# TUM-DAML/gemnet_pytorch

Hardware: AMD Instinct MI355X
Metric: molecules/sec (forward+force) GemNet-T on COLL-shaped batches (higher is better)
Workload: dtype f32

## Files before the change

gemnet_pytorch_amd/csrc/atom_stack.hip:

```cpp
#include <type_traits>

#include "common.h"

#include "chain_split.h"

#pragma clang fp contract(off)

#ifndef AS_EXP
#define AS_EXP 0
#endif

#ifndef AS_AHEAD
#define AS_AHEAD 2
#endif

namespace {
using namespace gn_split;

__device__ __forceinline__ float as_fma(float a, float b, float c) { return __builtin_fmaf(a, b, c); }

__device__ __forceinline__ void as_ssilu_pair(float x, float& y, float& d) {
  const float s = gn_sigmoid(x), xs = x * s;
  const float t = s + xs;
  d = as_fma(-s, xs, t) * GN_INV_06;
// ... 33 lines not shown

  uint4 w[NG][4][2];
  auto wload = [&](auto jc) {
    constexpr int j = decltype(jc)::value;
    if constexpr (j < NG) {
      const uint4* __restrict__ const base = P.W[j] + (size_t)wave * (4 * 2 * 64) + lane;
#pragma unroll
      for (int c = 0; c < 4; ++c)
#pragma unroll
        for (int p = 0; p < 2; ++p) w[j][c][p] = AS_EXP == 1 ? make_uint4(0x3c003c00u + lane, 0u, 0u, 0u) : base[(c * 2 + p) * 64];
    }
  };
  const int lr = tid >> 5, lc = (tid & 31) << 2;
  float4 xv = make_float4(0.f, 0.f, 0.f, 0.f);
  if (row0 + lr < M) xv = *reinterpret_cast<const float4*>(P.x + (size_t)(row0 + lr) * SW + lc);
  wload(std::integral_constant<int, 0>{});
  if constexpr (AS_AHEAD > 1) wload(std::integral_constant<int, 1>{});
  if constexpr (AS_AHEAD > 2) wload(std::integral_constant<int, 2>{});
  if constexpr (AS_AHEAD > 3) wload(std::integral_constant<int, 3>{});
  if constexpr (AS_AHEAD > 4) wload(std::integral_constant<int, 4>{});
  if constexpr (AS_AHEAD > 5) wload(std::integral_constant<int, 5>{});
  if constexpr (AS_AHEAD > 6) wload(std::integral_constant<int, 6>{});

  auto plane_ptr = [&](int slot, int p) -> unsigned char* { return smem + slot * SLOT + p * PLANE; };
  auto sw_off = [&](int row, int col) -> int { return row * ROWB + ((((col >> 3) ^ row) & 15) << 4) + ((col & 4) << 1); };
  auto slot_write = [&](int slot, int row, int col, const float4 v) {
    const int off = sw_off(row, col);
    uint2 H, Lo;
    split4h(v, H, Lo);
    *reinterpret_cast<uint2*>(plane_ptr(slot, 0) + off) = H;
    *reinterpret_cast<uint2*>(plane_ptr(slot, 1) + off) = Lo;
  };

  slot_write(0, lr, lc, xv);
  lds_barrier();

  const int n0 = wave * 16 + (lg << 2);
  const bool ok = row0 + l15 < M;
  const uint32_t off = (uint32_t)(row0 + l15) * (uint32_t)SW + (uint32_t)n0;
  const int my = sw_off(l15, n0);

  auto gemm = [&](auto jc) {
    constexpr int j = decltype(jc)::value;
    constexpr bool tail = j >= NM;
    constexpr bool second = !tail && j > 0 && (j & 1) == 0;
    constexpr bool last = j == NM - 1;
    constexpr int a_slot = tail ? 1 : (j & 1);
    constexpr int y_slot = a_slot ^ 1;
    uint4 xf[4][2];
    {
      const unsigned char* xb = smem + a_slot * SLOT + l15 * ROWB;
#pragma unroll
      for (int c = 0; c < 4; ++c) {
        const unsigned char* xp = xb + ((((c << 2) | lg) ^ l15) << 4);
        xf[c][0] = *reinterpret_cast<const uint4*>(xp);
        xf[c][1] = *reinterpret_cast<const uint4*>(xp + PLANE);
      }
    }
    uint2 rH = make_uint2(0u, 0u), rL = make_uint2(0u, 0u);
    if constexpr (second) {
      rH = *reinterpret_cast<const uint2*>(plane_ptr(y_slot, 0) + my);
      rL = *reinterpret_cast<const uint2*>(plane_ptr(y_slot, 1) + my);
    }
    float4 q2 = make_float4(0.f, 0.f, 0.f, 0.f);
    if constexpr (last && RES2) {
      if (ok) q2 = *reinterpret_cast<const float4*>(P.res2 + off);
    }
    v4f acc[3];
#pragma unroll
    for (int k = 0; k < 3; ++k) acc[k] = (v4f){0.f, 0.f, 0.f, 0.f};
#pragma unroll
    for (int c = 0; c < 4; ++c) {
      const f16x8 ah = __builtin_bit_cast(f16x8, w[j][c][0]), al = __builtin_bit_cast(f16x8, w[j][c][1]);
      const f16x8 yh = __builtin_bit_cast(f16x8, xf[c][0]), yl = __builtin_bit_cast(f16x8, xf[c][1]);
      if constexpr (AS_EXP == 3) {
        acc[0][0] += __uint_as_float(w[j][c][0].x ^ xf[c][0].x); acc[1][0] += __uint_as_float(w[j][c][0].y ^ xf[c][1].y);
        acc[2][0] += __uint_as_float(w[j][c][1].z ^ xf[c][0].z);
        continue;
      }
      acc[0] = __builtin_amdgcn_mfma_f32_16x16x32_f16(ah, yh, acc[0], 0, 0, 0);
      acc[1] = __builtin_amdgcn_mfma_f32_16x16x32_f16(ah, yl, acc[1], 0, 0, 0);
      acc[2] = __builtin_amdgcn_mfma_f32_16x16x32_f16(al, yh, acc[2], 0, 0, 0);
    }
    const v4f corr = acc[1] + acc[2];
    float4 v = make_float4(as_fma(corr[0], H_DOWN, acc[0][0]), as_fma(corr[1], H_DOWN, acc[0][1]),
                           as_fma(corr[2], H_DOWN, acc[0][2]), as_fma(corr[3], H_DOWN, acc[0][3]));
    wload(std::integral_constant<int, j + AS_AHEAD>{});
    if constexpr (tail) {
      if (ok) *reinterpret_cast<float4*>(P.t[j - NM] + off) = v;
    } else {
      float4 d;
      if constexpr (AS_EXP == 2) {
        d = v;
      } else {
        as_ssilu_pair(v.x, v.x, d.x); as_ssilu_pair(v.y, v.y, d.y);
        as_ssilu_pair(v.z, v.z, d.z); as_ssilu_pair(v.w, v.w, d.w);
      }
      if (ok) *reinterpret_cast<float4*>(P.z[j] + off) = d;
      if constexpr (second) {
        const float4 q = join4h(rH, rL);
        const float b = P.s;
        v.x = (v.x + q.x) * b; v.y = (v.y + q.y) * b; v.z = (v.z + q.z) * b; v.w = (v.w + q.w) * b;
      }
      if constexpr (last && RES2) {
        if (ok) {
          const float b = P.beta2;
          v.x = (v.x + q2.x) * b; v.y = (v.y + q2.y) * b; v.z = (v.z + q2.z) * b; v.w = (v.w + q2.w) * b;
        }
      }
      if constexpr (last) {
        if (ok) *reinterpret_cast<float4*>(P.y + off) = v;
      }
      if constexpr (!last || T > 0) {
        slot_write(y_slot, l15, n0, ok ? v : make_float4(0.f, 0.f, 0.f, 0.f));
        if constexpr (AS_EXP != 4) lds_barrier();
      }
    }
  };
  gemm(std::integral_constant<int, 0>{});
  if constexpr (NG > 1) gemm(std::integral_constant<int, 1>{});
  if constexpr (NG > 2) gemm(std::integral_constant<int, 2>{});
  if constexpr (NG > 3) gemm(std::integral_constant<int, 3>{});
  if constexpr (NG > 4) gemm(std::integral_constant<int, 4>{});
  if constexpr (NG > 5) gemm(std::integral_constant<int, 5>{});
  if constexpr (NG > 6) gemm(std::integral_constant<int, 6>{});
}

template <int L, int T, bool RES2>
int launch_fwd(const as_fwd_args& a, hipStream_t st) {
  hipLaunchKernelGGL((atom_stack_fwd_kernel<L, T, RES2>), dim3((unsigned)gn_cdiv(a.M, 16)), dim3(NT), 0, st, a);
  GN_LAUNCH_CHECK();
  return 0;
}

template <int L, int T>
int launch_fwd_res(const as_fwd_args& a, hipStream_t st) {
  if constexpr (L > 0) {
    if (a.res2) return launch_fwd<L, T, true>(a, st);
  }
  return launch_fwd<L, T, false>(a, st);
}

template <int L>
int launch_fwd_tails(const as_fwd_args& a, int tails, hipStream_t st) {
  switch (tails) {
    case 0: return launch_fwd_res<L, 0>(a, st);
    case 1: return launch_fwd_res<L, 1>(a, st);
    default: return launch_fwd_res<L, 2>(a, st);
  }
}

bool aligned16(const void* p) { return (reinterpret_cast<uintptr_t>(p) & 15u) == 0; }

}

extern "C" int gn_atom_stack_fwd_f32(const float* x, int M, int layers, int tails, const void* const* W, float* const* z,
                                     float s, const float* res2, float beta2, float* y, float* const* t, void* stream) {
  if (M <= 0) return 0;
  if (M > AS_MAX_ROWS || layers < 0 || layers > 2 || tails < 0 || tails > 2) return (int)hipErrorInvalidValue;
  if (!x || !y || !W || !z || (tails && !t) || (res2 && layers == 0)) return (int)hipErrorInvalidValue;
  if (!aligned16(x) || !aligned16(y) || !aligned16(res2)) return (int)hipErrorInvalidValue;
  as_fwd_args a = {};
  a.x = x; a.M = M; a.s = s; a.res2 = res2; a.beta2 = beta2; a.y = y;
  const int nm = 1 + 2 * layers;
  for (int j = 0; j < nm + tails; ++j) {
    if (!W[j] || !aligned16(W[j])) return (int)hipErrorInvalidValue;
    a.W[j] = static_cast<const uint4*>(W[j]);
  }
  for (int j = 0; j < nm; ++j) {
    if (!z[j] || !aligned16(z[j])) return (int)hipErrorInvalidValue;
    a.z[j] = z[j];
  }
  for (int j = 0; j < tails; ++j) {
    if (!t[j] || !aligned16(t[j])) return (int)hipErrorInvalidValue;
    a.t[j] = t[j];
  }
  hipStream_t st = static_cast<hipStream_t>(stream);
  switch (layers) {
    case 0: return launch_fwd_tails<0>(a, tails, st);
    case 1: return launch_fwd_tails<1>(a, tails, st);
    default: return launch_fwd_tails<2>(a, tails, st);
  }
}
```

gemnet_pytorch_amd/kernels.py:

```python
import contextlib
import ctypes
import functools
import os
import threading

import torch

from . import _lib
from ._lib import (GN_ANG_F16, GN_CHAIN_MAX_OPS, GN_CHAIN_ROW, GN_SPLIT_F16X2_ROW, GemmArgs, addr, check, ptr,
                   require_device, stream)


def _f32c(t):
    if t.dtype != torch.float32:
        raise TypeError(f"HIP path is fp32; got {t.dtype}")
    return t.contiguous()


def _rowmajor(t):
    if t.dtype != torch.float32:
        raise TypeError(f"HIP path is fp32; got {t.dtype}")
    if t.dim() != 2:
        raise ValueError("2-D operand expected")
    if t.shape[0] > 0 and t.shape[1] > 0 and t.stride(1) == 1 and t.stride(0) >= t.shape[1]:
# ... 1288 lines not shown


_CHAIN_PACK = None


def _chain_packer():
    global _CHAIN_PACK
    if _CHAIN_PACK is None:
        import struct
        from ._lib import ChainArgs, ChainOp
        code = {ctypes.c_int: "i", ctypes.c_float: "f", ctypes.c_void_p: "P"}
        names, fmt = [], "@"
        for name, ct in ChainOp._fields_:
            names.append(name)
            fmt += code[ct]
        st = struct.Struct(fmt)
        probe = bytearray(ctypes.sizeof(ChainOp))
        vals = list(range(1, len(names) + 1))
        st.pack_into(probe, 0, *[float(v) if c == ctypes.c_float else v for v, (_, c) in zip(vals, ChainOp._fields_)])
        chk = ChainOp.from_buffer_copy(bytes(probe))
        assert all(getattr(chk, n) == (float(v) if c == ctypes.c_float else v)
                   for v, (n, c) in zip(vals, ChainOp._fields_)) and st.size <= ctypes.sizeof(ChainOp)
        default = [0.0 if c == ctypes.c_float else 0 for _, c in ChainOp._fields_]
        for i, n in enumerate(names):
            globals()["F_" + n] = i
            if n in ("slot", "a_slot", "mul_slot", "res_slot", "res2_slot", "y2_slot"):
                default[i] = -1
        _CHAIN_PACK = (st, default, ChainArgs.ops.offset, ctypes.sizeof(ChainOp), ctypes.sizeof(ChainArgs),
                       struct.Struct("@ii"))
    return _CHAIN_PACK


def _mat(t, cols=None):
    if not (t.is_cuda and t.dtype == torch.float32 and t.dim() == 2 and t.is_contiguous()):
        require_device(t)
        raise AssertionError("chain operands: contiguous fp32 2-D")
    if cols is not None and t.shape[1] != cols:
        raise AssertionError((tuple(t.shape), cols))
    return addr(t)


def _source(v, src, stage, cols):
    v[F_src_stage], v[F_src_mode], v[F_src_alpha] = stage, int(src["mode"]), float(src["alpha"])
    v[F_srcP] = _mat(src["P"], cols)
    v[F_srcQ] = _mat(src["Q"], cols) if src["Q"] is not None else 0


GROUP_TILE_ROWS = int(os.environ.get("GN_CHAIN_GROUP_TILE_ROWS", "0"))


def pack_weight_split_stacked(Ws, trans=False, fmt=None):
    if fmt is None:
        fmt = split_format() or 0
    W0 = Ws[0]
    N, Kd = (W0.shape[1], W0.shape[0]) if trans else (W0.shape[0], W0.shape[1])
    nbytes = -(-N // 16) * -(-Kd // 32) * (2 if fmt else 3) * 64 * 16
    out = torch.empty((len(Ws), nbytes), device=W0.device, dtype=torch.uint8)
    for g, W in enumerate(Ws):
        require_device(W)
        W = _rowmajor(W)
        assert tuple(W.shape) == tuple(W0.shape)
        check(_lib.load().gn_pack_weight_split_fmt(ptr(W), N, Kd, W.stride(0), int(bool(trans)), int(fmt), ptr(out[g]), stream()),
              "gn_pack_weight_split_fmt")
    out._gn_fmt = fmt
    return out


def chain_grouped_supported(mode=None):
    return (mode or current_mode()) in ("h3", "split6") and CHAIN_LAYOUT == "tall"


USE_ATOM_STACK = os.environ.get("GEMNET_ATOM_STACK", "1") == "1"
ATOM_STACK_MAX_ROWS = 4096
ATOM_STACK_WIDTH = 128


def _atom_mat(t, M):
    return (torch.is_tensor(t) and t.dtype == torch.float32 and tuple(t.shape) == (M, ATOM_STACK_WIDTH)
            and t.is_contiguous() and t.data_ptr() % 16 == 0)


def _atom_gemm_plain(o):
    return (o["kind"] == "gemm" and tuple(o["W"].shape) == (ATOM_STACK_WIDTH, ATOM_STACK_WIDTH) and o["alpha"] == 1.0
            and o["gadd1"] is None and o["gadd2"] is None and o["mul"] is None and o["res_rows"] is None
            and o["y2"] < 0 and o["Z2"] is None and o["out2"] is None and o.get("add") is None and o.get("add2") is None)


def atom_stack_match(prog, mode=None):
    M, ops = prog.M, prog.ops
    if not (1 <= M <= ATOM_STACK_MAX_ROWS) or (mode or current_mode()) != "h3" or CHAIN_LAYOUT != "tall":
        return None
    if len(ops) < 2 or len(ops) > 8:
        return None
    o = ops[0]
    if not (o["kind"] == "load" and o["slot"] == 0 and o["rows"] is None and o.get("alpha", 1.0) == 1.0 and o.get("y2", -1) < 0
            and o.get("Z2") is None and o.get("add2") is None and _atom_mat(o["src"], M)):
        return None
    n_main = 0
    while 1 + n_main < len(ops) and ops[1 + n_main]["kind"] == "gemm" and ops[1 + n_main]["slot"] >= 0:
        n_main += 1
    main, tails = ops[1:1 + n_main], ops[1 + n_main:]
    L = (n_main - 1) // 2
    if n_main not in (1, 3, 5) or len(tails) > 2:
        return None
    s, res2, beta2 = 1.0, None, 1.0
    for j, g in enumerate(main):
        last = j + 1 == len(main)
        if not (_atom_gemm_plain(g) and g["act"] and g.get("pre_deriv") and _atom_mat(g["pre_out"], M)
                and g["a_slot"] == (j & 1) and g["slot"] == 1 - (j & 1)):
            return None
        if (g["out"] is not None) != last or (last and not _atom_mat(g["out"], M)):
            return None
        second = j > 0 and j % 2 == 0
        if second:
            if not (isinstance(g["res"], int) and g["res"] == 1 and (j == 2 or g["beta"] == s)):
                return None
            s = g["beta"]
        elif g["res"] is not None:
            return None
        if g["res2"] is not None:
            if not (second and last and _atom_mat(g["res2"], M)):
                return None
            res2, beta2 = g["res2"], g["beta2"]
    for g in tails:
        if not (_atom_gemm_plain(g) and not g["act"] and g["a_slot"] == 1 and g["slot"] < 0 and g["pre_out"] is None
                and g["res"] is None and g["res2"] is None and _atom_mat(g["out"], M)):
            return None
    return dict(x=ops[0]["src"], L=L, gemms=main + tails, z=[g["pre_out"] for g in main], s=s, res2=res2, beta2=beta2,
                y=main[-1]["out"], t=[g["out"] for g in tails])


def _atom_stack_fwd(M, m):
    fmt = SPLIT_FORMAT["h3"]
    require_device(m["x"], m["y"], m["res2"], *m["z"], *m["t"])
    Ws = []
    for g in m["gemms"]:
        Wp = g.get("packed")
        if Wp is None:
            _mat(g["W"])
            Wp = pack_weight_split(g["W"], fmt=fmt)
        elif getattr(Wp, "_gn_fmt", 0) != fmt:
            raise RuntimeError(f"chain: weight planes packed in format {getattr(Wp, '_gn_fmt', 0)} handed to a launch in "
                               f"mode 'h3' (format {fmt})")
        Ws.append(Wp)
    z, t = m["z"], m["t"]
    arr = ctypes.c_void_p
    check(_lib.load().gn_atom_stack_fwd_f32(ptr(m["x"]), int(M), int(m["L"]), len(t), (arr * len(Ws))(*[addr(W) for W in Ws]),
                                            (arr * len(z))(*[addr(a) for a in z]), float(m["s"]), ptr(m["res2"]),
                                            float(m["beta2"]), ptr(m["y"]), (arr * max(1, len(t)))(*[addr(a) for a in t]),
                                            stream()),
          "gn_atom_stack_fwd_f32")


def chain(prog, mode=None, groups=0, group_pitch=0, tile_rows=None):
    from ._lib import GN_OP_GEMM, GN_OP_LOAD, GN_OP_SCALE, GN_OP_STORE
    ops = prog.ops
    if len(ops) > GN_CHAIN_MAX_OPS:
        raise ValueError("chain program too long")
    mode = mode or current_mode()
    if USE_ATOM_STACK and not groups and prog.M <= ATOM_STACK_MAX_ROWS:
        m = atom_stack_match(prog, mode)
        if m is not None:
            return _atom_stack_fwd(prog.M, m)
    nprod = CHAIN_MODES[mode]
    if nprod and not chain_split_supported(prog):
        nprod = 0
    if groups and not (nprod and chain_grouped_supported(mode)):
        raise RuntimeError(f"chain: no grouped launch in mode {mode!r} / layout {CHAIN_LAYOUT!r} for this program")
    fmt = SPLIT_FORMAT.get(mode, 0)
    row = nprod == CHAIN_MODES["h3"] and CHAIN_LAYOUT == "row"
    if row and not chain_row_supported(prog):
        raise RuntimeError("chain: the row-resident layout needs K and every width to be a multiple of 16 "
                           "(GEMNET_CHAIN_LAYOUT=tall runs other shapes)")
    if row:
        fmt = GN_SPLIT_F16X2_ROW
    if nprod == CHAIN_MODES["h3"] and not row and h3_hazards(prog):
        raise RuntimeError("chain: this linear program adds a global tensor into an LDS-resident value "
                           f"(ops {h3_hazards(prog)}): not representable in the row-scaled fp16 form 'h3' — "
                           "launch it in kernels.linear_mode('h3')")
    st, default, ops_off, op_size, args_size, hdr = _chain_packer()
    keep = []
    buf = bytearray(args_size)
    M = prog.M
    hdr.pack_into(buf, 0, M, len(ops))
    has_src = False
    off = ops_off
    for o in ops:
        v = default[:]
        kind = o["kind"]
        if kind == "gemm":
            W = o["W"]
            N, Kd = W.shape
            if nprod:
                Wp = o.get("packed")
                if Wp is None:
                    _mat(W)
                    Wp = pack_weight_split(W, fmt=fmt)
                elif getattr(Wp, "_gn_fmt", 0) != fmt:
                    raise RuntimeError(f"chain: weight planes packed in format {getattr(Wp, '_gn_fmt', 0)} handed to a "
                                       f"launch in mode {mode!r} (format {fmt})")
                keep.append(Wp)
                v[F_W] = addr(Wp)
            else:
                v[F_W] = _mat(W)
            v[F_kind], v[F_N], v[F_K], v[F_a_slot], v[F_slot] = GN_OP_GEMM, N, Kd, o["a_slot"], o["slot"]
            v[F_act], v[F_alpha], v[F_beta], v[F_beta2] = int(o["act"]) | (2 if o.get("pre_deriv") else 0), o["alpha"], o["beta"], o["beta2"]
            if o.get("pre_deriv") and not nprod:
                raise RuntimeError("chain: pre_deriv needs the split-operand kernel (not CHAIN_MODE 'f32')")
            t = o["gadd1"]
            if t is not None:
                v[F_gadd1], v[F_gidx1] = _mat(t, N), addr(o["gidx1"])
            t = o["gadd2"]
            if t is not None:
                v[F_gadd2], v[F_gidx2] = _mat(t, N), addr(o["gidx2"])
            t = o["pre_out"]
            if t is not None:
                v[F_pre_out] = _mat(t, N)
            t = o["out"]
            if t is not None:
                v[F_out] = _mat(t, N)
            t = o["mul"]
            if t is not None:
                if isinstance(t, int):
                    v[F_mul_slot] = t
                else:
                    v[F_mul_g] = _mat(t, N)
            t = o["res"]
            if t is not None:
                if isinstance(t, int):
                    v[F_res_slot] = t
                else:
                    v[F_res_g] = _mat(t, N)
            t = o["res2"]
            if t is not None:
                if isinstance(t, int):
                    v[F_res2_slot] = t
                else:
                    v[F_res2_g] = _mat(t, N)
            t = o["res_rows"]
            if t is not None:
                v[F_res_rows] = addr(t)
            mm = o["mul_mode"]
            v[F_mul_mode], v[F_y2_slot], v[F_y2_src], v[F_mode2], v[F_alpha2] = mm, o["y2"], o["y2_src"], o["mode2"], o["alpha2"]
            t = o["Z2"]
            if t is not None:
                v[F_Z2] = _mat(t, N)
            t = o["out2"]
            if t is not None:
                v[F_out2] = _mat(t, N)
            if mm > 1:
                assert v[F_mul_slot] < 0 and v[F_mul_g], "mul_mode applies to a global mul operand"
            t = o.get("add")
            if t is not None:
                _source(v, t, 1, N)
                has_src = True
            t = o.get("add2")
            if t is not None:
                _source(v, t, 2, N)
                has_src = True
        elif kind == "load":
            src = o["src"]
            sp = _mat(src)
            assert o["rows"] is not None or src.shape[0] == M
            w = src.shape[1]
            v[F_kind], v[F_slot], v[F_width], v[F_ld], v[F_src] = GN_OP_LOAD, o["slot"], w, src.stride(0), sp
            t = o["rows"]
            if t is not None:
                v[F_rows] = addr(t)
            v[F_alpha], v[F_y2_slot], v[F_alpha2], v[F_mode2] = o.get("alpha", 1.0), o.get("y2", -1), o.get("alpha2", 1.0), o.get("mode2", 0)
            t = o.get("Z2")
            if t is not None:
                v[F_Z2] = _mat(t, w)
            t = o.get("add2")
            if t is not None:
                _source(v, t, 2, w)
                has_src = True
        elif kind == "scale":
            Z, out = o["Z"], o["out"]
            w = o["width"] or (Z.shape[1] if Z is not None else out.shape[1])
            v[F_kind], v[F_slot], v[F_a_slot], v[F_width], v[F_ld] = GN_OP_SCALE, o["slot"], o["a_slot"], w, w
            v[F_alpha], v[F_act] = o["alpha"], o.get("mode", 0)
            if Z is not None:
                v[F_src] = _mat(Z, w)
            if out is not None:
                v[F_out] = _mat(out, w)
            t = o.get("add")
            if t is not None:
                _source(v, t, 1, w)
                has_src = True
        else:
            out = o["out"]
            v[F_kind], v[F_slot], v[F_width], v[F_ld], v[F_out] = GN_OP_STORE, o["slot"], out.shape[1], out.stride(0), _mat(out)
        st.pack_into(buf, off, *v)
        off += op_size
    if has_src and not nprod:
        raise RuntimeError("chain programs with second-order source terms run on the split-operand kernel only "
                           "(CHAIN_MODE f32 / an unsupported shape): use the composite training path")
    cbuf = (ctypes.c_char * args_size).from_buffer(buf)
    if row:
        nprod |= GN_CHAIN_ROW
    if groups:
        if _lib.TRACE is not None:
            reads, writes = [], []
            for o in ops:
                for key, t in o.items():
                    if key == "packed" and t is not None:
                        reads.append((t.data_ptr(), t.numel() * t.element_size()))
                    elif torch.is_tensor(t) and key not in ("W", "packed") and t.dim() == 2:
                        span = ((int(groups) - 1) * int(group_pitch) + t.shape[0]) * t.stride(0) * t.element_size()
                        (writes if key in ("pre_out", "out", "out2") else reads).append((t.data_ptr(), span))
            _lib.note(reads=reads, writes=writes)
        check(_lib.load().gn_chain_split_grouped_f32(ctypes.addressof(cbuf), nprod, int(groups), int(group_pitch),
                                                     GROUP_TILE_ROWS if tile_rows is None else int(tile_rows), stream()),
              "gn_chain_split_grouped_f32")
    elif nprod:
        check(_lib.load().gn_chain_split_f32(ctypes.addressof(cbuf), nprod, stream()), "gn_chain_split_f32")
# ... 286 lines not shown
```

include/gemnet_hip.h:

```cpp
#ifndef GEMNET_HIP_H
#define GEMNET_HIP_H

#include <stdint.h>

#ifdef __cplusplus
extern "C" {
#endif

int gn_abi_version(void);
const char* gn_error_string(int code);

typedef struct {
  const float* A; const float* B; float* C;
  int M, N, K;
  int lda, ldb, ldc;
  int trans_a, trans_b;
  const float* a_dact_pre;
  int act;
  float* pre_out;
  const float* mul; int ldmul;
  float alpha;
  const float* res; int ldres;
  float beta;
  const float* gadd1; const int32_t* gidx1;
  const float* gadd2; const int32_t* gidx2;
  int ldg;
  const int32_t* ridx;
  const float* res2; int ldres2;
  float beta2;
  float* splitk_ws; int splitk;
} gn_gemm_args;
int gn_gemm_f32(const gn_gemm_args* args, void* stream);
int gn_gemm_f32_cfg(const gn_gemm_args* args, int cfg, void* stream);

enum { GN_OP_LOAD = 0, GN_OP_SCALE = 1, GN_OP_GEMM = 2, GN_OP_STORE = 3 };
#define GN_CHAIN_MAX_OPS 20
typedef struct {
  int kind;
  int slot;
  int a_slot;
  int width;
  int ld;
  const float* src;
  const int32_t* rows;
  const float* W; int N; int K;
  int act;
  float alpha;
  const float* gadd1; const int32_t* gidx1;
  const float* gadd2; const int32_t* gidx2;
  float* pre_out;
  int mul_slot; const float* mul_g;
  int res_slot; const float* res_g; const int32_t* res_rows; float beta;
  int res2_slot; const float* res2_g; float beta2;
  float* out;
  int mul_mode;
  int y2_slot;
  int y2_src;
  int mode2;
  float alpha2;
  const float* Z2;
  float* out2;
  int src_stage;
  int src_mode;
  float src_alpha;
  const float* srcP;
  const float* srcQ;
} gn_chain_op;
typedef struct {
  int M;
  int n_ops;
  gn_chain_op ops[GN_CHAIN_MAX_OPS];
} gn_chain_args;
int gn_chain_f32(const gn_chain_args* args, void* stream);

#define GN_CHAIN_F16X2 2
#define GN_CHAIN_ROW 0x200
int gn_chain_split_f32(const gn_chain_args* args, int nprod, void* stream);
#define GN_CHAIN_MAX_GROUPS 8
#define GN_CHAIN_GROUP_TILE_ROWS 32
int gn_chain_split_grouped_f32(const gn_chain_args* args, int nprod, int groups, int group_pitch, int tile_rows, void* stream);
int gn_atom_stack_fwd_f32(const float* x, int M, int layers, int tails, const void* const* W, float* const* z, float s,
                          const float* res2, float beta2, float* y, float* const* t, void* stream);
int gn_pack_weight_split(const float* W, int N, int K, int ldw, int trans, void* out, void* stream);
#define GN_SPLIT_BF16X3 0
#define GN_SPLIT_F16X2 1
#define GN_SPLIT_F16X2_ROW 2
int gn_pack_weight_split_fmt(const float* W, int N, int K, int ldw, int trans, int fmt, void* out, void* stream);
int64_t gn_pack_weight_split_bytes(int N, int K);
typedef struct {
  const float* W; void* out;
  int N, K, ldw, trans, unit_begin, fmt;
} gn_pack_job;
int gn_pack_weight_split_grouped(const gn_pack_job* jobs, int n_jobs, int total_units, void* stream);

int gn_gemm_tn_f32(const float* A, const float* B, float* C, int M, int N, int K, int lda, int ldb, int ldc,
                   float alpha, float* ws, int splitk, void* stream);
int gn_gemm_tn_splitk(int M, int N, int K);

typedef struct {
  const float* X; const float* Y;
  int M, N, K, ldx, ldy, splitk, kchunk, wg_begin;
  int64_t ws_off;
  float alpha;
  int pad_;
} gn_tn_problem;
typedef struct {
  float* out;
  int64_t n;
  int slice_begin, slice_end, wg_begin;
  int cols;
  int ld, pad_;
} gn_tn_target;
int gn_gemm_tn_grouped_f32(const gn_tn_problem* probs, int n_prob, int total_wg, const gn_tn_target* targets,
                           int n_target, int total_fold_wg, const int64_t* slice_off, float* ws, void* stream);

int gn_rbf_aggregate_fwd_f32(const float* m, const float* rbf, const float* W, const int32_t* perm, const int32_t* seg_off,
                             float* out, int64_t n_atoms, int C, int R, float scale, void* stream);
int gn_rbf_aggregate_bwd_f32(const float* g_out, const float* m, const float* rbf, const float* W, const int32_t* id_a,
                             float* g_m, float* g_rbf, int64_t E, int C, int R, float scale, int accum, void* stream);

#define GN_AGG_MAX_GROUPS 8
int gn_rbf_aggregate_grouped_fwd_f32(const float* const* m_list, const float* const* W_list, const float* scales, int G,
                                     const float* rbf, const int32_t* perm, const int32_t* seg_off, float* out, int64_t n_atoms,
                                     int C, int R, void* stream);
int gn_rbf_aggregate_grouped_bwd_f32(const float* g_out, const float* const* m_list, const float* const* W_list,
                                     const float* scales, int G, const float* rbf, const int32_t* id_a, float* const* g_m_list,
                                     float* g_rbf, int64_t E, int64_t n_atoms, int C, int R, int accum_m, int accum_rbf,
                                     void* stream);

int gn_energy_head_fwd_f32(const float* x, const float* w, float* E, int G, int64_t n_atoms, int C, void* stream);
int gn_energy_head_bwd_f32(const float* g_E, const float* w, float* g_x, int G, int64_t n_atoms, int C, void* stream);

int gn_quad_angles_fwd_f32(const float* R, const int32_t* qc, const int32_t* qa, const int32_t* qb, const int32_t* qd,
                           float* ang, int64_t Q, void* stream);
int gn_quad_angles_bwd_ld_f32(const float* g_ang, const float* R, const int32_t* qc, const int32_t* qa, const int32_t* qb,
                              const int32_t* qd, float* Gc, int ldc, float* Gb, int ldb, float* Gd, int ldd, int64_t Q,
                              void* stream);
#define GN_ANG_F16 1
int gn_bil_reduce_project_ang_f32(const float* ang, const float* x, const int32_t* expand_idx, const int32_t* seg_off,
                                  const float* B, float* Sm, float* P, int64_t E, int S, int C, int I, int arith,
                                  void* stream);
int gn_bil_expand_ang_f32(const float* ang, const float* dSm, const int32_t* seg_off, float* dxt, int64_t E, int S, int C,
                          int arith, void* stream);
int gn_bil_expand_rows_ang_f32(const float* ang, const float* dSm, const int32_t* a_perm, const int32_t* a_seg,
                               const int32_t* j_off, const int32_t* qmap, const int32_t* g_off, const int32_t* task_atom,
                               const int32_t* task_row0, int64_t n_tasks, float* dx, int S, int C, int arith, void* stream);
int gn_quad_angles_jvp_f32(const float* R, const float* tR, const int32_t* qc, const int32_t* qa, const int32_t* qb,
                           const int32_t* qd, float* tang, int64_t Q, void* stream);
int gn_bil_reduce_project_ang_tan_f32(const float* ang, const float* tang, const float* x, const float* tx,
                                      const int32_t* expand_idx, const int32_t* seg_off, const float* B, const float* tB,
                                      const float* Sm, float* Smd, float* Pd, int64_t E, int S, int C, int I, void* stream);
int gn_bil_expand_ang_tan_f32(const float* ang, const float* tang, const float* D1, const float* D2, const int32_t* seg_off,
                              float* dxt, int64_t E, int S, int C, void* stream);
int gn_bil_expand_rows_ang_tan_f32(const float* ang, const float* tang, const float* D1, const float* D2, const int32_t* a_perm,
                                   const int32_t* a_seg, const int32_t* j_off, const int32_t* qmap, const int32_t* g_off,
                                   const int32_t* task_atom, const int32_t* task_row0, int64_t n_tasks, float* dx, int S, int C,
                                   int tile, void* stream);
int gn_bil_dy_multi_ang_f32(const float* const* dSm_list, const float* const* x_list, int nb, const float* ang,
                            const int32_t* expand_idx, const int32_t* seg_off, float* g_ang, int64_t E, int S, int C,
                            int arith, void* stream);

int gn_bmm_f32(const float* A, const float* B, float* C, int batch, int m, int n, int k,
               int trans_a, int trans_b, void* stream);

int64_t gn_index_gpu_ws_bytes(int A, int64_t sum_n2, int triplets_only);
int gn_index_gpu_stage1(const void* R, int r_is_f64, const int32_t* mol_off, const int32_t* sq_off, int B, int A,
                        int nmax, int64_t sum_n2, double cutoff, double int_cutoff, int triplets_only, void* ws,
                        int32_t* batch_seg, int32_t* id_a, int32_t* id_c, int32_t* id_undir, int32_t* id_swap,
                        int32_t* id4_int_a, int32_t* id4_int_b, int64_t* sizes, void* stream);
int gn_index_gpu_stage2(const int32_t* mol_off, const int32_t* sq_off, int B, int A, int64_t sum_n2,
                        int triplets_only, void* ws, const int32_t* id_a, const int32_t* id_c,
                        const int32_t* id4_int_a, const int32_t* id4_int_b, int64_t E, int64_t Eint,
                        int32_t* id3_reduce_ca, int32_t* id3_expand_ba, int32_t* Kidx3, int32_t* id4_reduce_ca,
                        int32_t* id4_expand_db, int32_t* id4_reduce_cab, int32_t* id4_expand_abd, int32_t* Kidx4,
                        int32_t* id4_reduce_intm_ca, int32_t* id4_expand_intm_db, int32_t* id4_reduce_intm_ab,
                        int32_t* id4_expand_intm_ab, void* stream);

int gn_index_gpu_padded_t(const void* R, int r_is_f64, const int32_t* mol_off, const int32_t* sq_off, int B, int A, int nmax,
                          int64_t sum_n2, double cutoff, void* ws, int e_cap, int t_cap, int a_cap, int n_groups,
                          int deg_bound, int32_t* staging, int32_t* id_c, int32_t* id_a, int32_t* id_swap, int32_t* id_undir,
                          int32_t* id3_reduce_ca, int32_t* id3_expand_ba, int32_t* state, void* stream);
int gn_index_poison_f32(float* x, int64_t n, const int32_t* state, void* stream);
int gn_index_gpu_padded_q(const void* R, int r_is_f64, const int32_t* mol_off, const int32_t* sq_off, int B, int A, int nmax,
                          int64_t sum_n2, double cutoff, double int_cutoff, void* ws, int e_cap, int t_cap, int eint_cap,
                          int i_cap, int q_cap, int a_cap, int n_groups, int deg_bound, int32_t* staging, int32_t* const* arrays,
                          int32_t* state, void* stream);

int gn_gather_rows_f32(const float* x, const int32_t* idx, float* y, int64_t T, int C, void* stream);
int gn_gather_mul_f32(const float* x, const int32_t* idx, const float* m, float* y, int64_t T, int C, float scale,
                      void* stream);
int gn_segsum_rows_f32(const float* y, const int32_t* perm, const int32_t* seg_off, float* x,
                       int64_t N, int C, void* stream);
int gn_segsum_pair_f32(const float* y, const int32_t* perm1, const int32_t* seg_off1, float* x1, int64_t N1,
                       const int32_t* perm2, const int32_t* seg_off2, float* x2, int64_t N2, int C, void* stream);
int gn_segsum_multi_f32(int n_terms, const float* const* y, const int32_t* const* perm, const int32_t* const* seg_off,
                        const float* sign, float* x, int64_t N, int C, void* stream);

int64_t gn_csr_ws_bytes(int64_t n, int64_t n_rows);
int gn_csr_build_i32(const int32_t* keys, int64_t n, int64_t n_rows, int32_t* perm, int32_t* seg_off, void* ws,
                     int64_t ws_bytes, void* stream);
int gn_seg_offsets_i32(const int32_t* sorted_keys, int64_t n, int64_t n_rows, int32_t* seg_off, void* stream);
int gn_expanded_csr_i32(const int32_t* perm_e, const int32_t* seg_e, int64_t n_rows, const int32_t* seg_off_of_edge, int64_t E,
                        int32_t* perm, int32_t* seg_out, int32_t* ws, void* stream);

int gn_bil_reduce_f32(const float* Y, const float* x, const int32_t* expand_idx,
                      const int32_t* seg_off, float* Sm, int64_t E, int S, int C, void* stream);
int gn_bil_reduce_t_f32(const float* Y, const float* dSm, const int32_t* reduce_idx,
                        const int32_t* permT, const int32_t* segT_off, float* dx,
                        int64_t J, int S, int C, void* stream);
int gn_bil_reduce_t_grouped_f32(const float* Y, const float* dSm, const int32_t* grp_rows, const int32_t* grp_off,
                                const int32_t* grp_kseg, const int32_t* permT, const int32_t* rposT, float* dx,
                                int64_t G, int max_rows, int S, int C, void* stream);
int gn_bil_x_adjoint_atoms_f32(const float* Y, const float* dSm, const int32_t* grp_rows, const int32_t* grp_off,
                               const int32_t* grp_kseg, const int32_t* permT, const int32_t* rposT,
                               const int32_t* ent_off, const int32_t* ent_t, const int32_t* ent_bc, float* dx,
                               int64_t G, int max_rows, int S, int C, void* stream);
int gn_bil_expand_f32(const float* Y, const float* dSm, const int32_t* seg_off, float* dxt, int64_t E, int S, int C,
                      void* stream);
int gn_bil_dot_f32(const float* dSm, const float* x, const int32_t* expand_idx,
                   const int32_t* seg_off, float* dY, int64_t E, int S, int C, void* stream);

int gn_bil_reduce_project_f32(const float* Y, const float* x, const int32_t* expand_idx,
                              const int32_t* seg_off, const float* B, float* Sm, float* P, int64_t E, int S,
                              int C, int I, void* stream);
int gn_bil_reduce_project2_f32(const float* Y, const float* x, const int32_t* expand_idx, const int32_t* seg_off,
                               const float* B, const float* Sm_init, const float* B2, const float* Sm2, float* Sm, float* P,
                               int64_t E, int S, int C, int I, void* stream);
int gn_bil_fused_fwd_f32(const float* Y, const float* x, const int32_t* expand_idx, const int32_t* seg_off,
                         const float* B, const float* W2T, const void* W2T_planes, float* Sm, float* out, int64_t E, int S,
                         int C, int I, int O, float alpha, void* stream);
int gn_bil_up_fwd_f32(const float* Y, const float* x, const int32_t* expand_idx, const int32_t* seg_off, const float* B,
                      const void* W2T_planes, const void* Wup_planes, float* Sm, float* z_ac, float* z_ca, float* y_ac,
                      float* y_ca, int64_t E, int S, int C, int I, int O, int N_up, float alpha, float alpha_up, int act,
                      void* stream);
int gn_bil_project_bwd_f32(const float* dP, const float* Sm, const float* B, const float* x,
// ... 201 lines not shown
```

Measured before the change: 17810.

## Add fused atom-stack backward kernel matching adjoint chain programs

Adds a dedicated HIP kernel for the backward (adjoint) pass of the atom MLP stack. Each weight set stays in registers and activations stay in swizzled LDS fp16 hi/lo planes across all GEMMs, with MFMA 16x16x32 f16 split-precision products. The Python chain dispatcher pattern-matches adjoint programs (h3 mode, tall layout) and routes them to this kernel instead of the generic chain launcher. The goal is to cut launch overhead and global round-trips in the force backward, at the cost of a complex matcher that only covers specific program shapes.

After: 18370, median of 6. 1.03x the previous value.

```diff
diff --git a/gemnet_pytorch_amd/csrc/atom_stack.hip b/gemnet_pytorch_amd/csrc/atom_stack.hip
--- a/gemnet_pytorch_amd/csrc/atom_stack.hip
+++ b/gemnet_pytorch_amd/csrc/atom_stack.hip
@@ -209,6 +209,237 @@
 
 bool aligned16(const void* p) { return (reinterpret_cast<uintptr_t>(p) & 15u) == 0; }
 
+#ifndef AS_BWD_EXP
+#define AS_BWD_EXP 0
+#endif
+#ifndef AS_BWD_AHEAD
+#define AS_BWD_AHEAD 1
+#endif
+
+struct as_bwd_args {
+  const float* g;
+  const float* gt[2];
+  int M;
+  const uint4* W[AS_MAX_GEMMS];
+  const float* F[5];
+  float alpha0, a_out, a_s;
+  float bt[2], bl[2];
+  float* g_skip;
+  float* gx;
+};
+
+__device__ __forceinline__ float4 as_mul4(const float4 v, const float a) { return make_float4(v.x * a, v.y * a, v.z * a, v.w * a); }
+
+template <int L, int T, bool A>
+__global__ __launch_bounds__(NT) void atom_stack_bwd_kernel(const as_bwd_args P) {
+  static_assert(L >= 1 && L <= 2 && (T == 0 || T == 2), "adjoint programs of the atom stack");
+  constexpr int NG = T + 2 * L + 1;
+  constexpr int PLANE = 16 * ROWB;
+  constexpr int SLOT = 2 * PLANE;
+  __shared__ __attribute__((aligned(16))) unsigned char smem[4 * SLOT];
+  __shared__ float rs[3][16];
+  const int tid = threadIdx.x;
+  const int wave = tid >> 6;
+  const int lane = tid & 63;
+  const int l15 = lane & 15;
+  const int lg = lane >> 4;
+  const int M = P.M;
+  const int row0 = (int)blockIdx.x * 16;
+
+  uint4 w[NG][4][2];
+  auto wload = [&](auto jc) {
+    constexpr int j = decltype(jc)::value;
+    if constexpr (j < NG) {
+      const uint4* __restrict__ const base = P.W[j] + (size_t)wave * (4 * 2 * 64) + lane;
+#pragma unroll
+      for (int c = 0; c < 4; ++c)
+#pragma unroll
+        for (int p = 0; p < 2; ++p) w[j][c][p] = AS_BWD_EXP == 1 ? make_uint4(0x3c003c00u + lane, 0u, 0u, 0u) : base[(c * 2 + p) * 64];
+    }
+  };
+  auto plane_ptr = [&](int buf, int p) -> unsigned char* { return smem + buf * SLOT + p * PLANE; };
+  auto sw_off = [&](int row, int col) -> int { return row * ROWB + ((((col >> 3) ^ row) & 15) << 4) + ((col & 4) << 1); };
+  auto put_planes = [&](int buf, int off, const uint2 H, const uint2 Lo) {
+    *reinterpret_cast<uint2*>(plane_ptr(buf, 0) + off) = H;
+    *reinterpret_cast<uint2*>(plane_ptr(buf, 1) + off) = Lo;
+  };
+  auto sigma_of = [&](const float4 v) -> float {
+    if constexpr (AS_BWD_EXP == 3) return 1.f;
+    const float m = fmaxf(fmaxf(fabsf(v.x), fabsf(v.y)), fmaxf(fabsf(v.z), fabsf(v.w)));
+    return row_sigma(group_max(m, 32));
+  };
+  auto scale_read = [&](const uint2 H, const uint2 Lo, const float alpha, const float sc) -> float4 {
+    return as_mul4(join4h(H, Lo), alpha * inv_pow2(sc));
+  };
+
+  const int lr = tid >> 5, lc = (tid & 31) << 2;
+  const bool in = row0 + lr < M;
+  const size_t loff = (size_t)(row0 + lr) * SW + lc;
+  float4 gv = make_float4(0.f, 0.f, 0.f, 0.f), tv0 = gv, tv1 = gv, zv = gv;
+  if (in) {
+    gv = *reinterpret_cast<const float4*>(P.g + loff);
+    if constexpr (T > 0) tv0 = *reinterpret_cast<const float4*>(P.gt[0] + loff);
+    if constexpr (T > 1) tv1 = *reinterpret_cast<const float4*>(P.gt[1] + loff);
+    if constexpr (T == 0) zv = AS_BWD_EXP == 2 ? make_float4(1.f, 1.f, 1.f, 1.f) : *reinterpret_cast<const float4*>(P.F[0] + loff);
+  }
+  wload(std::integral_constant<int, 0>{});
+  if constexpr (AS_BWD_AHEAD > 1) wload(std::integral_constant<int, 1>{});
+  if constexpr (AS_BWD_AHEAD > 2) wload(std::integral_constant<int, 2>{});
+  {
+    const int o = sw_off(lr, lc);
+    const float4 v = as_mul4(gv, P.alpha0);
+    const float sig = sigma_of(v);
+    uint2 H, Lo;
+    split4h(as_mul4(v, sig), H, Lo);
+    if (lc == 0) rs[0][lr] = sig;
+    if constexpr (T == 0) {
+      if constexpr (A) {
+        float4 u = scale_read(H, Lo, P.a_out, sig);
+        if (in) *reinterpret_cast<float4*>(P.g_skip + loff) = u;
+        split4h(as_mul4(u, sig), H, Lo);
+        u = scale_read(H, Lo, P.a_s, sig);
+        split4h(as_mul4(u, sig), H, Lo);
+        put_planes(0, o, H, Lo);
+        u = scale_read(H, Lo, 1.f, sig);
+        if (in) { u.x *= zv.x; u.y *= zv.y; u.z *= zv.z; u.w *= zv.w; }
+        split4h(as_mul4(u, sig), H, Lo);
+        put_planes(1, o, H, Lo);
+      } else {
+        put_planes(0, o, H, Lo);
+        float4 u = v;
+        if (in) { u.x *= zv.x; u.y *= zv.y; u.z *= zv.z; u.w *= zv.w; }
+        split4h(as_mul4(u, sig), H, Lo);
+        put_planes(1, o, H, Lo);
+      }
+    } else {
+      put_planes(0, o, H, Lo);
+      const float s0 = sigma_of(tv0);
+      split4h(as_mul4(tv0, s0), H, Lo);
+      put_planes(1, o, H, Lo);
+      if (lc == 0) rs[1][lr] = s0;
+      if constexpr (T > 1) {
+        const float s1 = sigma_of(tv1);
+        split4h(as_mul4(tv1, s1), H, Lo);
+        put_planes(2, o, H, Lo);
+        if (lc == 0) rs[2][lr] = s1;
+      }
+    }
+  }
+  lds_barrier();
+
+  const int n0 = wave * 16 + (lg << 2);
+  const bool ok = row0 + l15 < M;
+  const uint32_t off = (uint32_t)(row0 + l15) * (uint32_t)SW + (uint32_t)n0;
+  const int my = sw_off(l15, n0);
+  uint2 GH = *reinterpret_cast<const uint2*>(plane_ptr(0, 0) + my), GL = *reinterpret_cast<const uint2*>(plane_ptr(0, 1) + my);
+  float rs0 = rs[0][l15], rs1 = rs0;
+
+  auto gemm = [&](auto jc) {
+    constexpr int j = decltype(jc)::value;
+    constexpr bool tail = j < T;
+    constexpr bool fin = j == NG - 1;
+    constexpr int m = j - T;
+    constexpr bool mulop = !tail && !fin && (m & 1) == 0;
+    constexpr bool resop = tail || (!fin && (m & 1) == 1);
+    constexpr bool scales = tail && j == T - 1 && A;
+    constexpr bool second = resop && !scales && !(tail && j < T - 1);
+    constexpr int fi = tail ? 0 : 1 + m;
+    constexpr bool factor = mulop || second || scales;
+    constexpr int a_buf = 1 + j % 3, y_buf = 1 + (j + 1) % 3;
+    uint4 xf[4][2];
+    {
+      const unsigned char* xb = smem + a_buf * SLOT + l15 * ROWB;
+#pragma unroll
+      for (int c = 0; c < 4; ++c) {
+        const unsigned char* xp = xb + ((((c << 2) | lg) ^ l15) << 4);
+        xf[c][0] = *reinterpret_cast<const uint4*>(xp);
+        xf[c][1] = *reinterpret_cast<const uint4*>(xp + PLANE);
+      }
+    }
+    float sa = rs1;
+    if constexpr (tail) sa = rs[1 + j][l15];
+    float4 fz = mulop ? make_float4(1.f, 1.f, 1.f, 1.f) : make_float4(0.f, 0.f, 0.f, 0.f);
+    if constexpr (factor) {
+      if (ok) fz = AS_BWD_EXP == 2 ? make_float4(1.f, 1.f, 1.f, 1.f) : *reinterpret_cast<const float4*>(P.F[fi] + off);
+    }
+    v4f acc[3];
+#pragma unroll
+    for (int k = 0; k < 3; ++k) acc[k] = (v4f){0.f, 0.f, 0.f, 0.f};
+#pragma unroll
+    for (int c = 0; c < 4; ++c) {
+      const f16x8 ah = __builtin_bit_cast(f16x8, w[j][c][0]), al = __builtin_bit_cast(f16x8, w[j][c][1]);
+      const f16x8 yh = __builtin_bit_cast(f16x8, xf[c][0]), yl = __builtin_bit_cast(f16x8, xf[c][1]);
+      acc[0] = __builtin_amdgcn_mfma_f32_16x16x32_f16(ah, yh, acc[0], 0, 0, 0);
+      acc[1] = __builtin_amdgcn_mfma_f32_16x16x32_f16(ah, yl, acc[1], 0, 0, 0);
+      acc[2] = __builtin_amdgcn_mfma_f32_16x16x32_f16(al, yh, acc[2], 0, 0, 0);
+    }
+    const v4f corr = acc[1] + acc[2];
+    float4 v = make_float4(as_fma(corr[0], H_DOWN, acc[0][0]), as_fma(corr[1], H_DOWN, acc[0][1]),
+                           as_fma(corr[2], H_DOWN, acc[0][2]), as_fma(corr[3], H_DOWN, acc[0][3]));
+    wload(std::integral_constant<int, j + AS_BWD_AHEAD>{});
+    v = as_mul4(v, inv_pow2(sa));
+    if constexpr (fin) {
+      if (ok) *reinterpret_cast<float4*>(P.gx + off) = v;
+    } else if constexpr (mulop) {
+      v.x *= fz.x; v.y *= fz.y; v.z *= fz.z; v.w *= fz.w;
+      uint2 H, Lo;
+      split4h(ok ? as_mul4(v, sa) : make_float4(0.f, 0.f, 0.f, 0.f), H, Lo);
+      put_planes(y_buf, my, H, Lo);
+      rs1 = sa;
+      if constexpr (AS_BWD_EXP != 4) lds_barrier();
+    } else {
+      const float sy = fminf(sa, rs0);
+      const float4 q = as_mul4(join4h(GH, GL), inv_pow2(rs0));
+      const float b = tail ? P.bt[tail ? j : 0] : P.bl[tail ? 0 : (m >> 1)];
+      v.x = (v.x + q.x) * b; v.y = (v.y + q.y) * b; v.z = (v.z + q.z) * b; v.w = (v.w + q.w) * b;
+      if constexpr (scales) {
+        if (ok) *reinterpret_cast<float4*>(P.g_skip + off) = v;
+      }
+      split4h(ok ? as_mul4(v, sy) : make_float4(0.f, 0.f, 0.f, 0.f), GH, GL);
+      rs0 = sy;
+      if constexpr (scales) {
+        float4 u = scale_read(GH, GL, P.a_s, sy);
+        split4h(as_mul4(u, sy), GH, GL);
+        u = scale_read(GH, GL, 1.f, sy);
+        if (ok) { u.x *= fz.x; u.y *= fz.y; u.z *= fz.z; u.w *= fz.w; }
+        uint2 H, Lo;
+        split4h(as_mul4(u, sy), H, Lo);
+        put_planes(y_buf, my, H, Lo);
+      } else if constexpr (second) {
+        float4 u = fz;
+        u.x *= v.x; u.y *= v.y; u.z *= v.z; u.w *= v.w;
+        uint2 H, Lo;
+        split4h(ok ? as_mul4(u, sy) : make_float4(0.f, 0.f, 0.f, 0.f), H, Lo);
+        put_planes(y_buf, my, H, Lo);
+      }
+      if constexpr (scales || second) {
+        rs1 = sy;
+        if constexpr (AS_BWD_EXP != 4) lds_barrier();
+      }
+    }
+  };
+  gemm(std::integral_constant<int, 0>{});
+  gemm(std::integral_constant<int, 1>{});
+  gemm(std::integral_constant<int, 2>{});
+  if constexpr (NG > 3) gemm(std::integral_constant<int, 3>{});
+  if constexpr (NG > 4) gemm(std::integral_constant<int, 4>{});
+  if constexpr (NG > 5) gemm(std::integral_constant<int, 5>{});
+  if constexpr (NG > 6) gemm(std::integral_constant<int, 6>{});
+}
+
+template <int L, int T, bool A>
+int launch_bwd(const as_bwd_args& a, hipStream_t st) {
+  hipLaunchKernelGGL((atom_stack_bwd_kernel<L, T, A>), dim3((unsigned)gn_cdiv(a.M, 16)), dim3(NT), 0, st, a);
+  GN_LAUNCH_CHECK();
+  return 0;
+}
+
+template <int L>
+int launch_bwd_form(const as_bwd_args& a, int tails, int form, hipStream_t st) {
+  if (tails == 0) return form ? launch_bwd<L, 0, true>(a, st) : launch_bwd<L, 0, false>(a, st);
+  return form ? launch_bwd<L, 2, true>(a, st) : launch_bwd<L, 2, false>(a, st);
+}
+
 }
 
 extern "C" int gn_atom_stack_fwd_f32(const float* x, int M, int layers, int tails, const void* const* W, float* const* z,
@@ -239,3 +470,29 @@
     default: return launch_fwd_tails<2>(a, tails, st);
   }
 }
+
+extern "C" int gn_atom_stack_bwd_f32(const float* g, int M, int layers, int tails, int form, const float* const* gt,
+                                     const void* const* W, const float* const* F, float alpha0, float a_out, float a_s, float bt0,
+                                     float bt1, float bl0, float bl1, float* g_skip, float* gx, void* stream) {
+  if (M <= 0) return 0;
+  if (M > AS_MAX_ROWS || layers < 1 || layers > 2 || (tails != 0 && tails != 2) || form < 0 || form > 1) return (int)hipErrorInvalidValue;
+  if (!g || !gx || !W || !F || (tails && !gt) || (form == 1) != (g_skip != nullptr)) return (int)hipErrorInvalidValue;
+  if (!aligned16(g) || !aligned16(gx) || !aligned16(g_skip)) return (int)hipErrorInvalidValue;
+  as_bwd_args a = {};
+  a.g = g; a.M = M; a.alpha0 = alpha0; a.a_out = a_out; a.a_s = a_s; a.g_skip = g_skip; a.gx = gx;
+  a.bt[0] = bt0; a.bt[1] = bt1; a.bl[0] = bl0; a.bl[1] = bl1;
+  for (int j = 0; j < tails; ++j) {
+    if (!gt[j] || !aligned16(gt[j])) return (int)hipErrorInvalidValue;
+    a.gt[j] = gt[j];
+  }
+  for (int j = 0; j < tails + 2 * layers + 1; ++j) {
+    if (!W[j] || !aligned16(W[j])) return (int)hipErrorInvalidValue;
+    a.W[j] = static_cast<const uint4*>(W[j]);
+  }
+  for (int j = 0; j < 2 * layers + 1; ++j) {
+    if (!F[j] || !aligned16(F[j])) return (int)hipErrorInvalidValue;
+    a.F[j] = F[j];
+  }
+  hipStream_t st = static_cast<hipStream_t>(stream);
+  return layers == 1 ? launch_bwd_form<1>(a, tails, form, st) : launch_bwd_form<2>(a, tails, form, st);
+}
diff --git a/gemnet_pytorch_amd/kernels.py b/gemnet_pytorch_amd/kernels.py
--- a/gemnet_pytorch_amd/kernels.py
+++ b/gemnet_pytorch_amd/kernels.py
@@ -1464,6 +1464,116 @@
           "gn_atom_stack_fwd_f32")
 
 
+USE_ATOM_STACK_BWD = os.environ.get("GEMNET_ATOM_STACK_BWD", "1") == "1"
+
+
+def _atom_adj_gemm(o):
+    return (o["kind"] == "gemm" and tuple(o["W"].shape) == (ATOM_STACK_WIDTH, ATOM_STACK_WIDTH) and not o["act"]
+            and not o.get("pre_deriv") and o["alpha"] == 1.0 and o["a_slot"] == 1 and o["pre_out"] is None
+            and o["gadd1"] is None and o["gadd2"] is None and o["res_rows"] is None and o["res2"] is None
+            and o["out2"] is None and o.get("add") is None and o.get("add2") is None and o["alpha2"] == 1.0 and o["y2_src"] == 0)
+
+
+def _atom_adj_res(o, M):
+    return (_atom_adj_gemm(o) and o["slot"] == 0 and o["mul"] is None and type(o["res"]) is int and o["res"] == 0)
+
+
+def _atom_adj_second(o, M):
+    return _atom_adj_res(o, M) and o["out"] is None and o["y2"] == 1 and o["mode2"] == 1 and _atom_mat(o["Z2"], M)
+
+
+def _atom_adj_scale(o, dst, M, Z=False, out=False):
+    return (o["kind"] == "scale" and o["slot"] == dst and o["a_slot"] == 0 and o["width"] in (None, ATOM_STACK_WIDTH)
+            and o.get("add") is None and (_atom_mat(o["Z"], M) and o.get("mode", 0) == 1 and o["alpha"] == 1.0 if Z else o["Z"] is None)
+            and (_atom_mat(o["out"], M) if out else o["out"] is None))
+
+
+def atom_stack_adjoint_match(prog, mode=None):
+    M, ops = prog.M, prog.ops
+    if not (1 <= M <= ATOM_STACK_MAX_ROWS) or (mode or current_mode()) != "h3" or CHAIN_LAYOUT != "tall":
+        return None
+    if not (4 <= len(ops) <= 12) or any(o["kind"] == "store" for o in ops):
+        return None
+
+    def plain_load(o, slot):
+        return (o["kind"] == "load" and o["slot"] == slot and o["rows"] is None and o.get("add2") is None and _atom_mat(o["src"], M)
+                and o.get("alpha", 1.0) == 1.0 and o.get("y2", -1) < 0 and o.get("Z2") is None)
+    o = ops[0]
+    m = dict(g=None, gt=[], gemms=[], F=[], form=0, alpha0=1.0, a_out=1.0, a_s=1.0, bt=[1.0, 1.0], bl=[1.0, 1.0], g_skip=None, gx=None)
+    i = 1
+    if plain_load(o, 0):
+        if plain_load(ops[1], 1):
+            if not (len(ops) >= 8 and _atom_adj_res(ops[2], M) and ops[2]["out"] is None and ops[2]["y2"] < 0 and ops[2]["Z2"] is None
+                    and plain_load(ops[3], 1) and _atom_adj_res(ops[4], M)):
+                return None
+            m["gt"], m["gemms"], m["bt"] = [ops[1]["src"], ops[3]["src"]], [ops[2], ops[4]], [ops[2]["beta"], ops[4]["beta"]]
+            t = ops[4]
+            if _atom_adj_second(t, M):
+                m["F"].append(t["Z2"])
+                i = 5
+            elif (_atom_mat(t["out"], M) and t["y2"] < 0 and t["Z2"] is None and _atom_adj_scale(ops[5], 0, M)
+                  and _atom_adj_scale(ops[6], 1, M, Z=True)):
+                m.update(form=1, g_skip=t["out"], a_s=ops[5]["alpha"])
+                m["F"].append(ops[6]["Z"])
+                i = 7
+            else:
+                return None
+        elif (_atom_adj_scale(ops[1], 0, M, out=True) and _atom_adj_scale(ops[2], 0, M) and _atom_adj_scale(ops[3], 1, M, Z=True)):
+            m.update(form=1, g_skip=ops[1]["out"], a_out=ops[1]["alpha"], a_s=ops[2]["alpha"])
+            m["F"].append(ops[3]["Z"])
+            i = 4
+        else:
+            return None
+    elif (o["kind"] == "load" and o["slot"] == 0 and o["rows"] is None and o.get("add2") is None and _atom_mat(o["src"], M)
+          and o.get("y2", -1) == 1 and o.get("alpha2", 1.0) == 1.0 and o.get("mode2", 0) == 1 and _atom_mat(o.get("Z2"), M)):
+        m["alpha0"] = o.get("alpha", 1.0)
+        m["F"].append(o["Z2"])
+    else:
+        return None
+    m["g"] = o["src"]
+    main = ops[i:]
+    L = (len(main) - 1) // 2
+    if len(main) not in (3, 5):
+        return None
+    for k in range(L):
+        a, b = main[2 * k], main[2 * k + 1]
+        if not (_atom_adj_gemm(a) and a["slot"] == 1 and a["res"] is None and a["out"] is None and a["y2"] < 0 and a["Z2"] is None
+                and a["mul_mode"] == 1 and _atom_mat(a["mul"], M) and _atom_adj_second(b, M)):
+            return None
+        m["F"] += [a["mul"], b["Z2"]]
+        m["bl"][k] = b["beta"]
+    f = main[-1]
+    if not (_atom_adj_gemm(f) and f["slot"] < 0 and f["mul"] is None and f["res"] is None and f["y2"] < 0 and f["Z2"] is None
+            and _atom_mat(f["out"], M)):
+        return None
+    m["gemms"] = m["gemms"] + list(main)
+    m.update(L=L, gx=f["out"])
+    return m
+
+
+def _atom_stack_bwd(M, m):
+    fmt = SPLIT_FORMAT["h3"]
+    require_device(m["g"], m["gx"], m["g_skip"], *m["gt"], *m["F"])
+    Ws = []
+    for g in m["gemms"]:
+        Wp = g.get("packed")
+        if Wp is None:
+            _mat(g["W"])
+            Wp = pack_weight_split(g["W"], fmt=fmt)
+        elif getattr(Wp, "_gn_fmt", 0) != fmt:
+            raise RuntimeError(f"chain: weight planes packed in format {getattr(Wp, '_gn_fmt', 0)} handed to a launch in "
+                               f"mode 'h3' (format {fmt})")
+        Ws.append(Wp)
+    gt, F = m["gt"], m["F"]
+    arr = ctypes.c_void_p
+    check(_lib.load().gn_atom_stack_bwd_f32(ptr(m["g"]), int(M), int(m["L"]), len(gt), int(m["form"]),
+                                            (arr * max(1, len(gt)))(*[addr(a) for a in gt]), (arr * len(Ws))(*[addr(W) for W in Ws]),
+                                            (arr * len(F))(*[addr(a) for a in F]), float(m["alpha0"]), float(m["a_out"]),
+                                            float(m["a_s"]), float(m["bt"][0]), float(m["bt"][1]), float(m["bl"][0]),
+                                            float(m["bl"][1]), ptr(m["g_skip"]), ptr(m["gx"]), stream()),
+          "gn_atom_stack_bwd_f32")
+
+
 def chain(prog, mode=None, groups=0, group_pitch=0, tile_rows=None):
     from ._lib import GN_OP_GEMM, GN_OP_LOAD, GN_OP_SCALE, GN_OP_STORE
     ops = prog.ops
@@ -1474,6 +1584,10 @@
         m = atom_stack_match(prog, mode)
         if m is not None:
             return _atom_stack_fwd(prog.M, m)
+    if USE_ATOM_STACK_BWD and not groups and prog.M <= ATOM_STACK_MAX_ROWS:
+        m = atom_stack_adjoint_match(prog, mode)
+        if m is not None:
+            return _atom_stack_bwd(prog.M, m)
     nprod = CHAIN_MODES[mode]
     if nprod and not chain_split_supported(prog):
         nprod = 0
diff --git a/include/gemnet_hip.h b/include/gemnet_hip.h
--- a/include/gemnet_hip.h
+++ b/include/gemnet_hip.h
@@ -81,6 +81,9 @@
 int gn_chain_split_grouped_f32(const gn_chain_args* args, int nprod, int groups, int group_pitch, int tile_rows, void* stream);
 int gn_atom_stack_fwd_f32(const float* x, int M, int layers, int tails, const void* const* W, float* const* z, float s,
                           const float* res2, float beta2, float* y, float* const* t, void* stream);
+int gn_atom_stack_bwd_f32(const float* g, int M, int layers, int tails, int form, const float* const* gt, const void* const* W,
+                          const float* const* F, float alpha0, float a_out, float a_s, float bt0, float bt1, float bl0, float bl1,
+                          float* g_skip, float* gx, void* stream);
 int gn_pack_weight_split(const float* W, int N, int K, int ldw, int trans, void* out, void* stream);
 #define GN_SPLIT_BF16X3 0
 #define GN_SPLIT_F16X2 1
```
